# reesque/SfmFromScratch

Measured on AMD Instinct MI355X. Metric: images/sec detect+describe+match, 1080p, 1/2/4/8 MI355X, higher is better.
Workload: dtype f32; 1 GPU; BASELINE configs[1]: 32x 1080p per GPU, ScaleRotInvSIFT 4-level x2 octave pyramid, k=2500, fw 18, NNRatio 0.85 over consecutive pairs; frames_per_gpu=32, pairs_per_gpu=31, distinct_batches=2, parallelism=image-shard x1, batches_in_flight=2

## Files before the change

include/sfmfeat.h:

```cpp
#ifndef SFMFEAT_H_
#define SFMFEAT_H_

#include <stddef.h>
#include <stdint.h>

#ifdef __cplusplus
extern "C" {
#endif

#define SFM_OK 0
#define SFM_EINVAL 1
#define SFM_ESTATE 2
#define SFM_EDEVICE 3
#define SFM_ERANGE 4
#define SFM_EINDEX 5

#define SFM_MODE_SCALEROT 0
#define SFM_MODE_NAIVE 1

#define SFM_DESC_DIM 128
#define SFM_MAX_GAUSS 15
#define SFM_MAX_KSIZE 31
#define SFM_MAX_FW 64
#define SFM_MAX_LEVELS 12
// ... 198 lines not shown

int32_t sfm_debug_nms(int32_t device, const float* R, int32_t B, int32_t H, int32_t W, int32_t ksize,
                      const uint32_t* tnms, int32_t tile, uint64_t* keys_out, int64_t* counts_out);

float sfm_debug_time_harris(int32_t device, int32_t abl, int32_t B, int32_t H, int32_t W,
                            int32_t iters);
float sfm_debug_harris_stamps(int32_t device, int32_t abl, int32_t B, int32_t H, int32_t W,
                              int32_t iters, uint64_t* out, int64_t cap);

int64_t sfm_debug_match_stamps(uint64_t* out, int64_t cap);

int32_t sfm_debug_match_operands(sfm_ctx* ctx, int32_t slot, int64_t rows, uint16_t* hi, uint16_t* lo,
                                 float* norm2, float* rnorm, float* pmax);
int32_t sfm_debug_match_windows(sfm_ctx* ctx, int32_t pair, int64_t rows, int32_t* cand_n, float* cand_thr,
                                uint32_t* cand);

int32_t sfm_copy_wg(void* dst, const void* src, int64_t bytes, int32_t workgroups, void* stream);

int32_t sfm_debug_select_stats(sfm_ctx* ctx, int32_t* fallback_planes, int32_t* total_planes);
int32_t sfm_debug_pose_candidates(sfm_ctx* ctx, int32_t* cand_idx, int64_t entries);
int32_t sfm_debug_ransac_fits(sfm_ctx* ctx, double* F, int32_t* counts, int64_t entries);
int32_t sfm_debug_copy_level(sfm_ctx* ctx, int32_t l, int32_t what, float* out, void* stream);


#ifdef __cplusplus
}
#endif

#endif
```

sfmfromscratch_amd/_abi.py:

```python
from __future__ import annotations

import ctypes

import numpy as np

SFM_OK = 0
SFM_EINVAL = 1
SFM_ESTATE = 2
SFM_EDEVICE = 3
SFM_ERANGE = 4
SFM_EINDEX = 5

SFM_MODE_SCALEROT = 0
SFM_MODE_NAIVE = 1

SFM_DESC_DIM = 128
SFM_MAX_GAUSS = 15
SFM_MAX_KSIZE = 31
SFM_MAX_FW = 64
SFM_MAX_LEVELS = 12
SFM_BA_MAX_CAMERAS = 256
SFM_BA_MAX_POINTS = 1 << 24
SFM_BA_MAX_OBSERVATIONS = 1 << 26
SFM_TRACKS_MAX_NODES = 1 << 30

_vp = ctypes.c_void_p
TRACK_SIGNATURES = {
    "sfm_build_tracks_dev": (ctypes.c_int32, [_vp, _vp, ctypes.c_int32, ctypes.c_int64, _vp, ctypes.c_int32, _vp,
                                              _vp, _vp, ctypes.c_int32, _vp, _vp, _vp, _vp, _vp, _vp]),
    "sfm_triangulate_tracks_dev": (ctypes.c_int32, [_vp, _vp, _vp, _vp, ctypes.c_int32, ctypes.c_int32, _vp,
                                                    ctypes.c_int32, ctypes.c_int64, _vp, _vp, ctypes.c_int32, _vp,
                                                    _vp, _vp]),
}


MATCH_DEBUG_SIGNATURES = {
    "sfm_debug_match_operands": (ctypes.c_int32, [_vp, ctypes.c_int32, ctypes.c_int64, _vp, _vp, _vp, _vp, _vp]),
    "sfm_debug_match_windows": (ctypes.c_int32, [_vp, ctypes.c_int32, ctypes.c_int64, _vp, _vp, _vp]),
}
GEOM_DEBUG_SIGNATURES = {
    "sfm_debug_geom": (ctypes.c_int32, [ctypes.c_int32, ctypes.c_int32, _vp, ctypes.c_int64, _vp]),
}
(SFM_GEOM_RODRIGUES, SFM_GEOM_RODRIGUES_INV, SFM_GEOM_EIG3, SFM_GEOM_NULL4, SFM_GEOM_COMPOSE, SFM_GEOM_ROTATE,
 SFM_GEOM_WAVE_SUM, SFM_GEOM_BLOCK_SUM) = range(8)
GEOM_ROW_IN = (3, 9, 6, 16, 18, 12, 64, 512)
GEOM_ROW_OUT = (9, 3, 12, 4, 9, 3, 64, 512)
SFM_GEOM_MAX_ROWS = 1 << 20
MATCH_CAND_CAP = 256
MATCH_PREP_ROWS = 16


class SfmParams(ctypes.Structure):
    _fields_ = [
# ... 52 lines not shown
```

sfmfromscratch_amd/_native.py:

```python
from __future__ import annotations

import ctypes
import os
import sys
import threading

import numpy as np

from . import _abi
from ._abi import SfmParams

_HERE = os.path.dirname(os.path.abspath(__file__))
LIB_PATH = os.environ.get("SFMFEAT_LIB", os.path.join(_HERE, "lib", "libsfmfeat.so"))

_lib = None
_lib_lock = threading.Lock()

_fp = ctypes.POINTER(ctypes.c_float)
_i64p = ctypes.POINTER(ctypes.c_int64)
_i32p = ctypes.POINTER(ctypes.c_int32)
_u8p = ctypes.POINTER(ctypes.c_uint8)
_dp = ctypes.POINTER(ctypes.c_double)
_vp = ctypes.c_void_p

# ... 396 lines not shown
        pmax = np.empty((capP // _abi.MATCH_PREP_ROWS, 2), np.float32)
        check(self.lib.sfm_debug_match_operands(self.handle, int(slot), capP, hi.ctypes.data, lo.ctypes.data,
                                                norm2.ctypes.data, rnorm.ctypes.data, pmax.ctypes.data),
              self.handle)
        return hi, lo, norm2, rnorm, pmax

    def match_windows(self, pair: int, rows: int):
        rows = int(rows)
        cn = np.empty(max(rows, 1), np.int32)
        ct = np.empty(max(rows, 1), np.float32)
        cd = np.empty((max(rows, 1), _abi.MATCH_CAND_CAP), np.uint32)
        check(self.lib.sfm_debug_match_windows(self.handle, int(pair), rows, cn.ctypes.data, ct.ctypes.data,
                                               cd.ctypes.data), self.handle)
        return cn, ct, cd

    def _tensor_ptr(self, t, dtype: str, numel: int, what: str, optional: bool = False):
        if t is None:
            if optional:
                return None
            raise ValueError(f"{what} is required")
        if not (hasattr(t, "data_ptr") and hasattr(t, "is_cuda")):
            raise ValueError(f"{what} must be a device tensor")
        if not t.is_cuda or (t.device.index or 0) != self.device:
            raise ValueError(f"{what} must live on cuda:{self.device} (the context's device), not {t.device}")
        if str(t.dtype) != "torch." + dtype:
            raise ValueError(f"{what} must be {dtype}, not {t.dtype}")
        if not t.is_contiguous():
            raise ValueError(f"{what} must be contiguous")
        if t.numel() < numel:
            raise ValueError(f"{what} has {t.numel()} elements, fewer than {numel}")
# ... 200 lines not shown
```

sfmfromscratch_amd/csrc/api_match.hip:

```cpp
#include "ctx.h"

using namespace sfm;

namespace {

constexpr int kFusedPrepSpare = 8;

int64_t operand_rows(const sfm_ctx* c, int64_t cap) {
  return c->match.direct ? (cap + 63) / 64 * 64 : (cap + 127) / 128 * 128;
}

int operands_claim(sfm_ctx* c, const float* desc, const int32_t* count, int64_t cap, int nimg) {
  MatchOperandsWs& o = c->match.ops;
  const int64_t capP = operand_rows(c, cap);
  const size_t rows = (size_t)nimg * capP;
  struct {
    DevBuf& b;
    size_t bytes;
  } mfma[] = {{o.hi, rows * 128 * 2}, {o.lo, rows * 128 * 2}, {o.norm2, rows * 4}, {o.rnorm, rows * 4},
              {o.imgmax, (size_t)nimg * match_pmax_bytes(capP)}},
    direct[] = {{o.descT, rows * 128 * 4}};
  bool fits = true;
  if (c->match.direct) {
    for (auto& e : direct) fits = fits && e.b.bytes >= e.bytes;
// ... 51 lines not shown
               const int32_t* pairs, int P, float ratio, int32_t* matches, float* conf,
               int32_t* nmatch, hipStream_t st, bool prep = true) {
  if (P <= 0) return SFM_OK;
  if (cap < 1 || cap > kMaxMatchRows)
    return set_err(c, SFM_EINVAL, "match capacity must be in [1, 16384]");
  int rc;
  MatchWs& m = c->match;
  MatchOperandsWs& o = m.ops;
  if (prep) {
    if ((rc = match_prep_range(c, desc, count, nimg, cap, 0, nimg, st, true))) return rc;
  } else {
    if (o.desc != desc || o.count != count || o.prep_nimg != nimg || o.cap != cap)
      return set_err(c, SFM_ESTATE, "sfm_match_pairs_prepped_dev: this table was not the last one prepped "
                                    "(sfm_match_prep_dev) on this context");
  }
  const size_t per_pair = (size_t)cap * (sizeof(RowBest) + sizeof(int2) + (m.direct ? 0 : kMatchCandCap * 4 + 8));
  const int Pmax = (int)std::max<size_t>(
      1, std::min<size_t>(std::min<size_t>((size_t)P, m.budget / per_pair), (size_t)1 << kMatchUnitPairBits));
  if ((rc = ensure(c, m.rows, (size_t)Pmax * cap * sizeof(RowBest)))) return rc;
  if ((rc = ensure(c, m.ovf, (size_t)Pmax * cap * sizeof(int2)))) return rc;
  if (m.ovfc.bytes == 0) {
    if ((rc = ensure(c, m.ovfc, 16))) return rc;
    HIPCHK(c, hipMemsetAsync(m.ovfc.p, 0, 16, st));
  }
  if (!m.direct) {
    if ((rc = ensure(c, m.cand, (size_t)Pmax * cap * kMatchCandCap * 4))) return rc;
    if ((rc = ensure(c, m.candn, (size_t)Pmax * cap * 4))) return rc;
    if ((rc = ensure(c, m.candt, (size_t)Pmax * cap * 4))) return rc;
    if ((rc = ensure(c, m.units, match_units_words(Pmax, (int)cap) * 4))) return rc;
  }
  const int64_t capP = operand_rows(c, cap);
  const bool skip_sweep = (extract_switches().skip & 8) != 0;
  m.last_P = P;
  m.last_cap = cap;
  m.last_subs = (P + Pmax - 1) / Pmax;
  for (int p0 = 0; p0 < P; p0 += Pmax, ++m.calls) {
    const int Pn = std::min(Pmax, P - p0);
    const int32_t* pr = pairs + 2 * (int64_t)p0;
    {
      StageScope sc(c, SFM_PROF_MATCH, st);
      if (m.direct)
        launch_match_rows(as<float>(o.descT), count, capP, pr, Pn, ratio, as<RowBest>(m.rows), (int)cap, st);
      else if (!(m.calls > 0 && skip_sweep))
        launch_match_mfma(desc, count, cap, capP, as<_Float16>(o.hi), as<_Float16>(o.lo), as<float>(o.norm2),
                          as<float>(o.rnorm), o.imgmax.p, pr, Pn, ratio, as<RowBest>(m.rows), (int)cap,
                          as<uint32_t>(m.cand), as<int32_t>(m.candn), as<float>(m.candt), as<int>(m.ovfc),
                          as<int2>(m.ovf), as<int32_t>(m.units), st);
    }
    {
      StageScope sc(c, SFM_PROF_MATCH_POST, st);
      launch_match_compact(as<RowBest>(m.rows), count, pr, Pn, (int)cap, cap, matches + (int64_t)p0 * cap * 2,
                           conf + (int64_t)p0 * cap, nmatch + p0, m.direct ? nullptr : as<int>(m.ovfc), st);
    }
  }
  HIPCHK(c, hipGetLastError());
  return SFM_OK;
}

}

int operands_fused_begin(sfm_ctx* c, const float* desc, const int32_t* count, int64_t cap, int B,
                         MatchOperands* mo) {
// ... 115 lines not shown
  MatchWs& m = c->match;
  if (m.direct) return set_err(c, SFM_ESTATE, "the direct matcher keeps no windows");
  if (m.last_subs != 1)
    return set_err(c, SFM_ESTATE, m.last_subs ? "the last match call ran as more than one sub-launch"
                                              : "no match call on this context yet");
  if (pair >= m.last_P || rows > m.last_cap) return set_err(c, SFM_EINVAL, "pair or rows outside the last match call");
  HIPCHK(c, hipSetDevice(c->device));
  HIPCHK(c, hipDeviceSynchronize());
  const size_t r0 = (size_t)pair * (size_t)m.last_cap, n = (size_t)rows;
  HIPCHK(c, hipMemcpy(cand_n, as<int32_t>(m.candn) + r0, n * 4, hipMemcpyDeviceToHost));
  HIPCHK(c, hipMemcpy(cand_thr, as<float>(m.candt) + r0, n * 4, hipMemcpyDeviceToHost));
  HIPCHK(c, hipMemcpy(cand, as<uint32_t>(m.cand) + r0 * kMatchCandCap, n * kMatchCandCap * 4, hipMemcpyDeviceToHost));
  return SFM_OK;
}

}
```

sfmfromscratch_amd/csrc/ctx.h:

```cpp
#pragma once

#include <stdlib.h>
#include <string.h>

#include <algorithm>
#include <string>
#include <utility>
#include <vector>

#include "../../include/sfmfeat.h"
#include "extract_layout.h"
#include "kernels.h"

struct DevBuf {
  void* p = nullptr;
  size_t bytes = 0;
  DevBuf() = default;
  DevBuf(const DevBuf&) = delete;
  DevBuf& operator=(const DevBuf&) = delete;
  DevBuf(DevBuf&& o) noexcept : p(o.p), bytes(o.bytes) { o.p = nullptr, o.bytes = 0; }
  DevBuf& operator=(DevBuf&& o) noexcept {
    if (this != &o) {
      release();
      std::swap(p, o.p);
// ... 59 lines not shown
  int last_B = 0, last_H = 0, last_W = 0;
};

struct MatchOperandsWs {
  DevBuf hi, lo, norm2, rnorm, imgmax;
  DevBuf descT;
  const float* desc = nullptr;
  const int32_t* count = nullptr;
  int64_t cap = -1;
  int fused_B = 0;
  int prep_nimg = -1;
};

struct MatchWs {
  MatchOperandsWs ops;
  DevBuf rows, ovf, ovfc, cand, candn, candt, units;
  DevBuf h_desc, h_count, h_pairs, h_matches, h_conf, h_nmatch;
  bool fused_prep = false;
  bool direct = false;
  size_t budget = (size_t)4096 << 20;
  int64_t calls = 0;
  int last_P = 0, last_subs = 0;
  int64_t last_cap = 0;
};

struct IngestWs {
  DevBuf tab_h, tab_v, tmp, rgb, gray;
  DevBuf colmap, sets;
  int w = -1, w2 = -1, h = -1, h2 = -1, ksh = 0, ksv = 0, nsets = 0;
  bool rows = false;
  std::vector<int32_t> th, tv;
// ... 146 lines not shown
```

sfmfromscratch_amd/csrc/kernels.h:

```cpp
#pragma once

#include <hip/hip_runtime.h>
#include <stdint.h>

#include <vector>

#include "common.h"

namespace sfm {

#define SFM_NMS_MAX_HALF 15

constexpr int kHistBits = 12;
constexpr int kHistBins = 1 << kHistBits;
constexpr int kMedBits1 = 11;
constexpr int kMedBins1 = 1 << kMedBits1;
constexpr int kTopkLdsCap = 8192;
constexpr int kMaxMatchRows = 16384;
constexpr int kMatchCandCap = 256;
constexpr int kCounterStride = 32;
constexpr int kMatchUnitPairBits = 20;

constexpr float kMatchScale = 256.0f;
constexpr float kMatchLoScale = 2048.0f;
// ... 322 lines not shown
void launch_transpose_desc(const float* desc, const int32_t* count, int nimg, int64_t cap,
                           int64_t capP, float* descT, hipStream_t st);
void launch_match_rows(const float* descT, const int32_t* count, int64_t capP, const int32_t* pairs,
                       int P, float ratio, RowBest* rows, int max_rows, hipStream_t st);
void launch_match_compact(const RowBest* rows, const int32_t* count, const int32_t* pairs, int P,
                          int max_rows, int64_t cap, int32_t* matches, float* conf, int32_t* nmatch,
                          int* reset_counter, hipStream_t st);
void init_match_attributes(int max_rows);
size_t match_pmax_bytes(int64_t capP);
void launch_match_prep(const float* desc, const int32_t* count, int nimg, int64_t cap, int64_t capP,
                       _Float16* hi, _Float16* lo, float* norm2, float* rnorm, void* pmax, hipStream_t st);
void launch_match_mfma(const float* desc, const int32_t* count, int64_t cap, int64_t capP,
                       const _Float16* hi, const _Float16* lo, const float* norm2, const float* rnorm,
                       const void* pmax, const int32_t* pairs, int P, float ratio,
                       RowBest* rows, int max_rows, uint32_t* cand, int32_t* cand_n, float* cand_thr,
                       int* ovf_count, int2* ovf_list, int32_t* units, hipStream_t st);

}
```

sfmfromscratch_amd/csrc/match_mfma.hip:

```cpp
#include <stdlib.h>

#include <type_traits>

#include "kernels.h"

namespace sfm {

typedef _Float16 h8 __attribute__((ext_vector_type(8)));
typedef float f32x16 __attribute__((ext_vector_type(16)));

constexpr int kQW = 32;
constexpr int kWaves = 8;
constexpr int kQB = kQW * kWaves;
constexpr int kNT = 64 * kWaves;
constexpr int kRowH = 128 + 8;
constexpr int kCandCap = kMatchCandCap;
constexpr int kHalfCap = kCandCap / 2;
constexpr float kScale = kMatchScale;
constexpr float kLoScale = kMatchLoScale;

__global__ void __launch_bounds__(256) k_match_prep(const float* __restrict__ desc,
                                                   const int32_t* __restrict__ count, int64_t cap,
                                                   int64_t capP, _Float16* __restrict__ hi,
                                                   _Float16* __restrict__ lo,
// ... 89 lines not shown

SFM_DEV float other_half(float x) {
  const auto r = __builtin_amdgcn_permlane32_swap(__float_as_uint(x), __float_as_uint(x), false, false);
  return __uint_as_float((threadIdx.x & 32) ? r[0] : r[1]);
}
SFM_DEV int other_half(int x) { return __float_as_int(other_half(__int_as_float(x))); }

SFM_DEV void top2_merge(float& b1, int& j1, float& b2, float ob1, int oj1, float ob2) {
  if (ob1 < b1 || (ob1 == b1 && oj1 < j1)) {
    b2 = fminf(b1, ob2);
    b1 = ob1;
    j1 = oj1;
  } else {
    b2 = fminf(b2, ob1);
  }
}

constexpr int kTT2 = 64;
constexpr int kDmaBufs = 3, kDmaNormBufs = 4;
constexpr int kRegBufs = 2, kRegNormBufs = 3;
constexpr size_t kDBytes = (size_t)kWaves * 64 * 16 * 4;
constexpr size_t kSweepLds = (size_t)kDmaBufs * 2 * kTT2 * 256 + kDmaNormBufs * kTT2 * 4 + kDBytes;
static_assert(kSweepLds >= (size_t)kRegBufs * 2 * kTT2 * kRowH * 2 + kRegNormBufs * kTT2 * 4 + kDBytes,
              "one LDS array serves both staging forms");
static_assert(kSweepLds <= 160 * 1024, "LDS per CU");
constexpr int kWaves3 = 4;
constexpr size_t kSweepLds3 = (size_t)2 * 2 * kTT2 * 256 + 3 * kTT2 * 4 + 256;
static_assert(kSweepLds3 <= 80 * 1024, "half-CU sweep: at most half of the CU's LDS");
constexpr int sweep_waves(int stage) { return stage == 3 ? kWaves3 : kWaves; }
constexpr int sweep_rows(int stage) { return kQW * sweep_waves(stage); }
// ... 3 lines not shown
  asm volatile("s_mov_b32 %0, m0\n\ts_mov_b32 m0, %2\n\ts_nop 0\n\tglobal_load_lds_dwordx4 %1, off\n\ts_mov_b32 m0, %0"
               : "=&s"(keep)
               : "v"(gsrc), "s"(lds_dst)
               : "memory");
}
__device__ __forceinline__ void glds_x1(const void* gsrc, uint32_t lds_dst) {
  uint32_t keep;
  asm volatile("s_mov_b32 %0, m0\n\ts_mov_b32 m0, %2\n\ts_nop 0\n\tglobal_load_lds_dword %1, off\n\ts_mov_b32 m0, %0"
               : "=&s"(keep)
               : "v"(gsrc), "s"(lds_dst)
               : "memory");
}

__global__ void __launch_bounds__(1024) k_match_units(const int32_t* __restrict__ count,
                                                      const int32_t* __restrict__ pairs, int P, int max_rows,
                                                      int qbr, int32_t* __restrict__ units) {
  __shared__ uint32_t s_w[16];
  const int tid = threadIdx.x, lane = tid & 63, wid = tid >> 6;
  uint32_t base = 0;
  for (int c0 = 0; c0 < P; c0 += 1024) {
    const int p = c0 + tid;
    uint32_t q = 0;
    if (p < P) {
      const int n1 = min(count[pairs[2 * p]], max_rows), n2 = count[pairs[2 * p + 1]];
      q = (n1 > 0 && n2 > 0) ? (uint32_t)((n1 + qbr - 1) / qbr) : 0u;
    }
    const uint32_t x = wave_inclusive_scan(q);
    if (lane == 63) s_w[wid] = x;
    __syncthreads();
    uint32_t before = 0, tot = 0;
    for (int w = 0; w < 16; ++w) {
      const uint32_t t = s_w[w];
      before += w < wid ? t : 0u;
      tot += t;
    }
    const uint32_t first = base + before + x - q;
    for (uint32_t j = 0; j < q; ++j) units[1 + first + j] = (int32_t)((uint32_t)p | (j << kMatchUnitPairBits));
    base += tot;
    __syncthreads();
  }
  if (tid == 0) units[0] = (int32_t)base;
}

constexpr int kStampWg = 16, kStampSt = 40;
__device__ uint64_t g_match_stamps[kStampWg][kWaves][kStampSt + 1][4];
constexpr int kStampAll = 1024;
__device__ uint64_t g_match_wg[kStampAll][4];

template <int STAGE, int ABL = 0>
__global__ void __launch_bounds__(64 * sweep_waves(STAGE), STAGE == 3 ? 2 : 1) k_match_mfma(
    const int32_t* __restrict__ count, int64_t capP, const _Float16* __restrict__ hi,
    const _Float16* __restrict__ lo, const float* __restrict__ norm2, const float* __restrict__ rnorm,
    const float2* __restrict__ pmax, const int32_t* __restrict__ pairs, int P, int max_rows,
    uint32_t* __restrict__ cand, int32_t* __restrict__ cand_n, float* __restrict__ cand_thr,
    int* __restrict__ ovf_count, int2* __restrict__ ovf_list, const int32_t* __restrict__ units) {
  constexpr bool DMA = STAGE >= 1;
  constexpr bool H3 = STAGE == 3;
  constexpr int NW = sweep_waves(STAGE), NTH = 64 * NW, QBR = sweep_rows(STAGE);
  constexpr int NBUF = H3 ? 2 : DMA ? kDmaBufs : kRegBufs;
  constexpr int NNB = H3 ? 3 : DMA ? kDmaNormBufs : kRegNormBufs;
  constexpr int ROWB = DMA ? 256 : kRowH * 2;
  constexpr int ARRB = kTT2 * ROWB;
  constexpr int BUFB = 2 * ARRB;
  constexpr int OFF_N = NBUF * BUFB;
  constexpr int OFF_D = OFF_N + NNB * kTT2 * 4;
  constexpr size_t LDSB = H3 ? kSweepLds3 : kSweepLds;
  static_assert((size_t)OFF_D + (H3 ? 256 : kDBytes) <= LDSB, "LDS carve");
  __shared__ __attribute__((aligned(16))) unsigned char smem[LDSB];
  float* const sNb = reinterpret_cast<float*>(smem + OFF_N);
  float* const sDb = reinterpret_cast<float*>(smem + OFF_D);
// ... 25 lines not shown
    p = code & ((1 << kMatchUnitPairBits) - 1);
    row0 = (code >> kMatchUnitPairBits) * QBR;
  } else {
    p = grp + 8 * (slot8 / QB);
    row0 = (slot8 % QB) * QBR;
    if (p >= P) return;
  }
  const int tid = threadIdx.x, lane = tid & 63, wid = tid >> 6;
  const int i1 = pairs[2 * p], i2 = pairs[2 * p + 1];
  const int n1 = count[i1], n2 = count[i2];
  if (row0 >= n1 || n2 < 1) return;

  const int ql = wid * kQW + (lane & 31);
  const int qi = row0 + ql;
  const int half = lane >> 5;
  const int64_t qo = ((int64_t)i1 * capP + qi) * 128;
  h8 qhi[8], qlo[8];
#pragma unroll
  for (int kk = 0; kk < 8; ++kk) {
    qhi[kk] = *reinterpret_cast<const h8*>(hi + qo + kk * 16 + 8 * half);
    qlo[kk] = *reinterpret_cast<const h8*>(lo + qo + kk * 16 + 8 * half);
  }
  const float na = norm2[(int64_t)i1 * capP + qi];
  const float ra = rnorm[(int64_t)i1 * capP + qi];
  float maxn2, maxrn;
  {
    const int nblk = (int)(capP / kPrepRows);
    float m2 = 0.0f, mr = 0.0f;
    for (int t = tid; t < nblk; t += NTH) {
      const float2 v = pmax[(int64_t)i2 * nblk + t];
      m2 = fmaxf(m2, v.x);
      mr = fmaxf(mr, v.y);
    }
    for (int off = 32; off >= 1; off >>= 1) {
      m2 = fmaxf(m2, __shfl_xor(m2, off));
      mr = fmaxf(mr, __shfl_xor(mr, off));
    }
    if (lane == 0) {
      sDb[2 * wid] = m2;
// ... 333 lines not shown
  if constexpr (DMA) asm volatile("s_waitcnt vmcnt(0)" ::: "memory");
  if constexpr (STAMP) {
    if (tid == 0 && blockIdx.x < kStampAll) {
      g_match_wg[blockIdx.x][1] = __builtin_amdgcn_s_memrealtime();
      g_match_wg[blockIdx.x][3] = (uint64_t)p | ((uint64_t)row0 << 32);
    }
    if (lane == 0) s_stamp[(wid * (kStampSt + 1) + kStampSt) * 4 + 2] = __builtin_amdgcn_s_memrealtime();
    if (blockIdx.x < kStampWg) {
      __builtin_amdgcn_s_waitcnt(0xc07f);
      const uint64_t* src = s_stamp + wid * (kStampSt + 1) * 4;
      uint64_t* dst = &g_match_stamps[blockIdx.x][wid][0][0];
      for (int i = lane; i < (kStampSt + 1) * 4; i += 64) dst[i] = src[i];
    }
  }
  const float ob1 = other_half(b1), ob2 = other_half(b2);
  const float thr_final = fminf(fminf(fmaxf(b1, ob1), fminf(b2, ob2)) + E2, thr_w);
  const int ocnt = other_half(cnt);
  const bool unbounded = !(E2 <= 3.0e38f);
  if (live && half == 0) {
    cand_thr[(int64_t)p * max_rows + qi] = thr_final;
    cand_n[(int64_t)p * max_rows + qi] = unbounded ? 0x7fff : cnt | (ocnt << 16);
    if (cnt > kHalfCap || ocnt > kHalfCap || unbounded) {
      const int k = atomicAdd(ovf_count, 1);
      ovf_list[k] = make_int2(p, qi);
    }
  }
}

__global__ void __launch_bounds__(256) k_match_rerank(const float* __restrict__ desc,
                                                      const int32_t* __restrict__ count, int64_t cap,
                                                      const int32_t* __restrict__ pairs, int P, float ratio,
                                                      int max_rows, const uint32_t* __restrict__ cand,
                                                      const int32_t* __restrict__ cand_n,
                                                      const float* __restrict__ cand_thr,
                                                      RowBest* __restrict__ rows_out) {
  __shared__ uint16_t sJ[4][kCandCap];
  const int lane = threadIdx.x & 63, wv = threadIdx.x >> 6;
  const int grp = lane >> 3, l8 = lane & 7;
  const int64_t w = (int64_t)blockIdx.x * 4 + wv;
  const int p = (int)(w / max_rows), row = (int)(w % max_rows);
  if (p >= P) return;
  const int i1 = pairs[2 * p], i2 = pairs[2 * p + 1];
  const int n1 = count[i1], n2 = count[i2];
  if (row >= n1 || n2 < 1) return;
  const int cw = cand_n[w];
  const int c0 = cw & 0xffff, c1 = cw >> 16;
  if (c0 > kHalfCap || c1 > kHalfCap) return;
  const float thr = cand_thr[w];
  const uint32_t* list = cand + w * kCandCap;
  const float* A = desc + ((int64_t)i1 * cap + row) * 128;
  const float* Bd = desc + (int64_t)i2 * cap * 128;
  float a[16];
#pragma unroll
  for (int i = 0; i < 16; ++i) a[i] = A[8 * i + l8];
  int nk = 0;
  static_assert(kHalfCap % 64 == 0, "whole wavefront passes per half-list");
#pragma unroll
  for (int h = 0; h < 2; ++h) {
    const int ch = h ? c1 : c0;
// ... 43 lines not shown
    const float d1 = sqrtf(e1), d2 = sqrtf(e2);
    if (d2 > 0.0f) {
      const float nndr = d1 / d2;
      if (nndr <= ratio) { rb.col = j1; rb.nndr = nndr; }
    }
    rows_out[w] = rb;
  }
}

__global__ void __launch_bounds__(256) k_match_rerank2(const float* __restrict__ desc,
                                                       const int32_t* __restrict__ count, int64_t cap,
                                                       const int32_t* __restrict__ pairs, int P, float ratio,
                                                       int max_rows, const uint32_t* __restrict__ cand,
                                                       const int32_t* __restrict__ cand_n,
                                                       const float* __restrict__ cand_thr,
                                                       RowBest* __restrict__ rows_out) {
  __shared__ uint16_t sJ[4][2][kCandCap];
  const int lane = threadIdx.x & 63, wv = threadIdx.x >> 6, hf = lane >> 5, hl = lane & 31;
  const int grp = hl >> 3, l8 = lane & 7;
  const int64_t w = ((int64_t)blockIdx.x * 4 + wv) * 2 + hf;
  const int p = (int)(w / max_rows), row = (int)(w % max_rows);
  bool ok = p < P;
  int i1 = 0, i2 = 0, n1 = 0, n2 = 0;
  if (ok) {
    i1 = pairs[2 * p];
    i2 = pairs[2 * p + 1];
    n1 = count[i1];
    n2 = count[i2];
    ok = row < n1 && n2 >= 1;
  }
  int c0 = 0, c1 = 0;
  float thr = 0.0f;
  if (ok) {
    const int cw = cand_n[w];
    c0 = cw & 0xffff;
    c1 = cw >> 16;
    ok = c0 <= kHalfCap && c1 <= kHalfCap;
    thr = cand_thr[w];
  }
  const uint32_t* list = cand + w * kCandCap;
  const float* A = desc + ((int64_t)i1 * cap + row) * 128;
  const float* Bd = desc + (int64_t)i2 * cap * 128;
  float a[16];
#pragma unroll
  for (int i = 0; i < 16; ++i) a[i] = ok ? A[8 * i + l8] : 0.0f;
// ... 53 lines not shown
      const float nndr = d1 / d2;
      if (nndr <= ratio) { rb.col = j1; rb.nndr = nndr; }
    }
    rows_out[w] = rb;
  }
}

constexpr int kRrRows = 8;
constexpr int kRerank8MaxPairs = 0;
__global__ void __launch_bounds__(256) k_match_rerank8(const float* __restrict__ desc,
                                                      const int32_t* __restrict__ count, int64_t cap,
                                                      const int32_t* __restrict__ pairs, int P, float ratio,
                                                      int max_rows, const uint32_t* __restrict__ cand,
                                                      const int32_t* __restrict__ cand_n,
                                                      const float* __restrict__ cand_thr,
                                                      RowBest* __restrict__ rows_out) {
  __shared__ __attribute__((aligned(16))) float sA[4][kRrRows][128];
  __shared__ uint16_t sL[4][kRrRows * kCandCap];
  __shared__ float sDist[4][kRrRows * kCandCap];
  __shared__ int sBeg[4][kRrRows + 1];
  const int lane = threadIdx.x & 63, wv = threadIdx.x >> 6;
  const int grp = lane >> 3, l8 = lane & 7;
  const int64_t total = (int64_t)P * max_rows;
  const int64_t w0 = ((int64_t)blockIdx.x * 4 + wv) * kRrRows;
  if (w0 >= total) return;
  int c_l = 0, ok_l = 0, i1_l = 0, i2_l = 0, row_l = 0, p_l = 0;
  float thr_l = 0.0f;
  if (lane < kRrRows) {
    const int64_t w = w0 + lane;
    if (w < total) {
      p_l = (int)(w / max_rows);
      row_l = (int)(w % max_rows);
      i1_l = pairs[2 * p_l];
      i2_l = pairs[2 * p_l + 1];
      const int n1 = count[i1_l], n2 = count[i2_l];
      if (row_l < n1 && n2 >= 1) {
        c_l = cand_n[w];
        thr_l = cand_thr[w];
        ok_l = ((c_l & 0xffff) <= kHalfCap && (c_l >> 16) <= kHalfCap) ? 1 : 0;
      }
    }
    if (!ok_l) c_l = 0;
  }
#pragma unroll
  for (int q = 0; q < 4; ++q) {
    const int e = lane * 4 + 256 * q;
    const int r = e >> 7, k = e & 127;
    const int ir = __shfl(i1_l, r), rr = __shfl(row_l, r), okr = __shfl(ok_l, r);
    float4 v = make_float4(0.0f, 0.0f, 0.0f, 0.0f);
    if (okr) v = *reinterpret_cast<const float4*>(desc + ((int64_t)ir * cap + rr) * 128 + k);
    *reinterpret_cast<float4*>(&sA[wv][r][k]) = v;
  }
  const uint32_t* lists = cand + w0 * kCandCap;
  int nk = 0;
#pragma unroll 4
  for (int sidx = 0; sidx < kRrRows * kCandCap / 64; ++sidx) {
    const int e = sidx * 64 + lane;
    const int r = e / kCandCap, pos = e % kCandCap;
    const int cr = __shfl(c_l, r);
    const float tr = __shfl(thr_l, r);
    const int crh = pos < kHalfCap ? (cr & 0xffff) : (cr >> 16);
    const bool valid = (pos & (kHalfCap - 1)) < crh && w0 + r < total;
    const uint32_t ent = valid ? lists[e] : 0u;
    const bool keep = valid && __uint_as_float(ent & 0xffff0000u) <= tr;
    const uint64_t bal = __ballot(keep);
    if (pos == 0 && lane == (sidx * 64) % 64 && (e % kCandCap) == 0) sBeg[wv][r] = nk;
    if (keep) sL[wv][nk + __popcll(bal & ((1ull << lane) - 1ull))] = (uint16_t)(ent & 0xffffu);
    nk += __popcll(bal);
  }
  if (lane == 0) sBeg[wv][kRrRows] = nk;
  __builtin_amdgcn_wave_barrier();
  for (int s0 = 0; s0 < nk; s0 += 8) {
    const int s = s0 + grp;
    const bool ok = s < nk;
    const int j = ok ? (int)sL[wv][s] : 0;
    int r = 0;
#pragma unroll
    for (int k = 1; k < kRrRows; ++k) r += (s >= sBeg[wv][k]) ? 1 : 0;
// ... 19 lines not shown
    const int beg = sBeg[wv][lane], end = lane + 1 < kRrRows ? sBeg[wv][lane + 1] : nk;
    for (int s = beg; s < end; ++s) {
      const float dd = sDist[wv][s];
      const int j = (int)sL[wv][s];
      if (dd < e1 || (dd == e1 && j < j1)) { e2 = e1; e1 = dd; j1 = j; }
      else if (dd < e2) e2 = dd;
    }
    RowBest rb;
    rb.col = -1;
    rb.nndr = 0.0f;
    const float d1 = sqrtf(e1), d2 = sqrtf(e2);
    if (d2 > 0.0f) {
      const float nndr = d1 / d2;
      if (nndr <= ratio) { rb.col = j1; rb.nndr = nndr; }
    }
    rows_out[w0 + lane] = rb;
  }
}

__global__ void __launch_bounds__(256) k_match_overflow(const float* __restrict__ desc,
                                                        const int32_t* __restrict__ count, int64_t cap,
                                                        const int32_t* __restrict__ pairs, float ratio,
                                                        RowBest* __restrict__ rows_out, int max_rows,
                                                        const int* __restrict__ ovf_count,
                                                        const int2* __restrict__ ovf_list) {
  const int nov = *ovf_count;
  const int lane = threadIdx.x & 63;
  for (int w = blockIdx.x * 4 + (threadIdx.x >> 6); w < nov; w += gridDim.x * 4) {
    const int2 ent = ovf_list[w];
    const int p = ent.x, row = ent.y;
    const int i1 = pairs[2 * p], i2 = pairs[2 * p + 1];
// ... 31 lines not shown
  return 1 + (size_t)P * ((max_rows + sweep_rows(3) - 1) / sweep_rows(3));
}

size_t match_pmax_bytes(int64_t capP) { return (size_t)(capP / kPrepRows) * sizeof(float2); }

void launch_match_prep(const float* desc, const int32_t* count, int nimg, int64_t cap, int64_t capP,
                       _Float16* hi, _Float16* lo, float* norm2, float* rnorm, void* pmax, hipStream_t st) {
  hipLaunchKernelGGL(k_match_prep, dim3((unsigned)(capP / kPrepRows), nimg), dim3(256), 0, st, desc, count, cap,
                     capP, hi, lo, norm2, rnorm, static_cast<float2*>(pmax));
}

void launch_match_mfma(const float* desc, const int32_t* count, int64_t cap, int64_t capP,
                       const _Float16* hi, const _Float16* lo, const float* norm2, const float* rnorm,
                       const void* pmax, const int32_t* pairs, int P, float ratio,
                       RowBest* rows, int max_rows, uint32_t* cand, int32_t* cand_n, float* cand_thr,
                       int* ovf_count, int2* ovf_list, int32_t* units, hipStream_t st) {
  static const int stage = [] {
    const char* e = getenv("SFMFEAT_MATCH_STAGE");
    return (e && e[0] == 'r') ? 0 : (e && e[0] == '1') ? 1 : 3;
  }();
  static const int rr8_max = [] {
    const char* e = SFM_DIAG_ENV("SFMFEAT_RERANK8_MAX");
    return e ? atoi(e) : kRerank8MaxPairs;
  }();
  static const bool use_units = [] {
    const char* e = SFM_DIAG_ENV("SFMFEAT_MATCH_UNITS");
    return !(e && e[0] == '0');
  }();
  const int qbr = stage == 3 ? sweep_rows(3) : kQB;
  const int qb = (max_rows + qbr - 1) / qbr;
  const dim3 grid((unsigned)(8 * ((P + 7) / 8) * qb));
  if (!use_units) units = nullptr;
  if (units) hipLaunchKernelGGL(k_match_units, dim3(1), dim3(1024), 0, st, count, pairs, P, max_rows, qbr, units);
#define SFM_SWEEP(A, ABL)                                                                             \
  hipLaunchKernelGGL((k_match_mfma<A, ABL>), grid, dim3(64 * sweep_waves(A)), 0, st, count, capP, hi, lo,  \
                     norm2, rnorm,                                                                         \
                     static_cast<const float2*>(pmax), pairs, P, max_rows, cand, cand_n, cand_thr, ovf_count, \
                     ovf_list, units)
  static const int abl = [] {
    const char* e = SFM_ABLATION_ENV("SFMFEAT_MATCH_ABL");
    return e ? atoi(e) : 0;
  }();
#ifdef SFM_ABLATIONS
  switch (abl) {
    case 1: SFM_SWEEP(1, 1); break;
    case 2: SFM_SWEEP(1, 2); break;
    case 3: SFM_SWEEP(1, 3); break;
    case 4: SFM_SWEEP(1, 4); break;
    case 6: SFM_SWEEP(1, 6); break;
    case 16: SFM_SWEEP(1, 16); break;
    case 17: SFM_SWEEP(1, 17); break;
    case 32: SFM_SWEEP(1, 32); break;
    default: if (stage == 0) SFM_SWEEP(0, 0); else if (stage == 3) SFM_SWEEP(3, 0); else SFM_SWEEP(1, 0);
// ... 2 lines not shown
  (void)abl;
  if (stage == 0)
    SFM_SWEEP(0, 0);
  else if (stage == 3)
    SFM_SWEEP(3, 0);
  else
    SFM_SWEEP(1, 0);
#endif
#undef SFM_SWEEP
  static const int rr2 = [] {
    const char* e = getenv("SFMFEAT_RERANK2");
    return e ? atoi(e) : 1;
  }();
  if (rr2 && P > rr8_max)
    hipLaunchKernelGGL(k_match_rerank2, dim3((unsigned)(((int64_t)P * max_rows + 7) / 8)), dim3(256), 0, st, desc,
                       count, cap, pairs, P, ratio, max_rows, cand, cand_n, cand_thr, rows);
  else if (P <= rr8_max)
    hipLaunchKernelGGL(k_match_rerank8, dim3((unsigned)(((int64_t)P * max_rows + 4 * kRrRows - 1) / (4 * kRrRows))),
                       dim3(256), 0, st, desc, count, cap, pairs, P, ratio, max_rows, cand, cand_n, cand_thr, rows);
  else
    hipLaunchKernelGGL(k_match_rerank, dim3((unsigned)(((int64_t)P * max_rows + 3) / 4)), dim3(256), 0, st, desc,
                       count, cap, pairs, P, ratio, max_rows, cand, cand_n, cand_thr, rows);
  hipLaunchKernelGGL(k_match_overflow, dim3(256), dim3(256), 0, st, desc, count, cap, pairs, ratio, rows, max_rows,
                     ovf_count, ovf_list);
}

int64_t match_stamps_copy(uint64_t* out, int64_t cap) {
#ifdef SFM_ABLATIONS
  const int64_t n1 = (int64_t)sizeof(g_match_stamps) / 8, n = n1 + (int64_t)sizeof(g_match_wg) / 8;
  if (cap < n) return -1;
  if (hipMemcpyFromSymbol(out, HIP_SYMBOL(g_match_stamps), sizeof(g_match_stamps)) != hipSuccess) return -1;
  if (hipMemcpyFromSymbol(out + n1, HIP_SYMBOL(g_match_wg), sizeof(g_match_wg)) != hipSuccess) return -1;
  return n;
#else
  (void)out;
  (void)cap;
  return -1;
// ... 5 lines not shown
```

Before: 43570 images/sec.

## Skip provably unmatched rows in sweep and compact rerank work list

The MFMA sweep now checks, using the sweep's approximate best and second-best distances and their error bound, whether a row cannot pass the ratio test; such rows get a no-match result written directly. Remaining rows are appended to a compacted work list through wave-level ballot and atomics, and the rerank kernels walk that list instead of every (pair,row) slot. This cuts exact rerank work and idle waves, at the cost of extra atomics, a per-row skip byte buffer, and indirect candidate loads. Rerank grids stay sized for the full row count, so the extra blocks exit early.

```diff
diff --git a/include/sfmfeat.h b/include/sfmfeat.h
--- a/include/sfmfeat.h
+++ b/include/sfmfeat.h
@@ -236,6 +236,7 @@
                                  float* norm2, float* rnorm, float* pmax);
 int32_t sfm_debug_match_windows(sfm_ctx* ctx, int32_t pair, int64_t rows, int32_t* cand_n, float* cand_thr,
                                 uint32_t* cand);
+int32_t sfm_debug_match_skips(sfm_ctx* ctx, int32_t pair, int64_t rows, uint8_t* skip);
 
 int32_t sfm_copy_wg(void* dst, const void* src, int64_t bytes, int32_t workgroups, void* stream);
 
diff --git a/sfmfromscratch_amd/_abi.py b/sfmfromscratch_amd/_abi.py
--- a/sfmfromscratch_amd/_abi.py
+++ b/sfmfromscratch_amd/_abi.py
@@ -37,6 +37,7 @@
 MATCH_DEBUG_SIGNATURES = {
     "sfm_debug_match_operands": (ctypes.c_int32, [_vp, ctypes.c_int32, ctypes.c_int64, _vp, _vp, _vp, _vp, _vp]),
     "sfm_debug_match_windows": (ctypes.c_int32, [_vp, ctypes.c_int32, ctypes.c_int64, _vp, _vp, _vp]),
+    "sfm_debug_match_skips": (ctypes.c_int32, [_vp, ctypes.c_int32, ctypes.c_int64, _vp]),
 }
 GEOM_DEBUG_SIGNATURES = {
     "sfm_debug_geom": (ctypes.c_int32, [ctypes.c_int32, ctypes.c_int32, _vp, ctypes.c_int64, _vp]),
diff --git a/sfmfromscratch_amd/_native.py b/sfmfromscratch_amd/_native.py
--- a/sfmfromscratch_amd/_native.py
+++ b/sfmfromscratch_amd/_native.py
@@ -434,6 +434,12 @@
                                                cd.ctypes.data), self.handle)
         return cn, ct, cd
 
+    def match_skips(self, pair: int, rows: int):
+        rows = int(rows)
+        sk = np.empty(max(rows, 1), np.uint8)
+        check(self.lib.sfm_debug_match_skips(self.handle, int(pair), rows, sk.ctypes.data), self.handle)
+        return sk
+
     def _tensor_ptr(self, t, dtype: str, numel: int, what: str, optional: bool = False):
         if t is None:
             if optional:
diff --git a/sfmfromscratch_amd/csrc/api_match.hip b/sfmfromscratch_amd/csrc/api_match.hip
--- a/sfmfromscratch_amd/csrc/api_match.hip
+++ b/sfmfromscratch_amd/csrc/api_match.hip
@@ -89,9 +89,11 @@
       return set_err(c, SFM_ESTATE, "sfm_match_pairs_prepped_dev: this table was not the last one prepped "
                                     "(sfm_match_prep_dev) on this context");
   }
-  const size_t per_pair = (size_t)cap * (sizeof(RowBest) + sizeof(int2) + (m.direct ? 0 : kMatchCandCap * 4 + 8));
+  const size_t per_pair = (size_t)cap * (sizeof(RowBest) + sizeof(int2) + (m.direct ? 0 : kMatchCandCap * 4 + 13));
   const int Pmax = (int)std::max<size_t>(
-      1, std::min<size_t>(std::min<size_t>((size_t)P, m.budget / per_pair), (size_t)1 << kMatchUnitPairBits));
+      1, std::min<size_t>(std::min<size_t>(std::min<size_t>((size_t)P, m.budget / per_pair),
+                                           (size_t)1 << kMatchUnitPairBits),
+                          (size_t)0x7fffffff / (size_t)cap));
   if ((rc = ensure(c, m.rows, (size_t)Pmax * cap * sizeof(RowBest)))) return rc;
   if ((rc = ensure(c, m.ovf, (size_t)Pmax * cap * sizeof(int2)))) return rc;
   if (m.ovfc.bytes == 0) {
@@ -102,6 +104,8 @@
     if ((rc = ensure(c, m.cand, (size_t)Pmax * cap * kMatchCandCap * 4))) return rc;
     if ((rc = ensure(c, m.candn, (size_t)Pmax * cap * 4))) return rc;
     if ((rc = ensure(c, m.candt, (size_t)Pmax * cap * 4))) return rc;
+    if ((rc = ensure(c, m.cands, (size_t)Pmax * cap))) return rc;
+    if ((rc = ensure(c, m.work, (size_t)Pmax * cap * 4))) return rc;
     if ((rc = ensure(c, m.units, match_units_words(Pmax, (int)cap) * 4))) return rc;
   }
   const int64_t capP = operand_rows(c, cap);
@@ -119,8 +123,8 @@
       else if (!(m.calls > 0 && skip_sweep))
         launch_match_mfma(desc, count, cap, capP, as<_Float16>(o.hi), as<_Float16>(o.lo), as<float>(o.norm2),
                           as<float>(o.rnorm), o.imgmax.p, pr, Pn, ratio, as<RowBest>(m.rows), (int)cap,
-                          as<uint32_t>(m.cand), as<int32_t>(m.candn), as<float>(m.candt), as<int>(m.ovfc),
-                          as<int2>(m.ovf), as<int32_t>(m.units), st);
+                          as<uint32_t>(m.cand), as<int32_t>(m.candn), as<float>(m.candt), as<uint8_t>(m.cands),
+                          as<uint32_t>(m.work), as<int>(m.ovfc), as<int2>(m.ovf), as<int32_t>(m.units), st);
     }
     {
       StageScope sc(c, SFM_PROF_MATCH_POST, st);
@@ -266,4 +270,19 @@
   return SFM_OK;
 }
 
-}
+int32_t sfm_debug_match_skips(sfm_ctx* c, int32_t pair, int64_t rows, uint8_t* skip) {
+  if (!c || !skip || pair < 0 || rows < 1) return SFM_EINVAL;
+  MatchWs& m = c->match;
+  if (m.direct) return set_err(c, SFM_ESTATE, "the direct matcher keeps no windows");
+  if (m.last_subs != 1)
+    return set_err(c, SFM_ESTATE, m.last_subs ? "the last match call ran as more than one sub-launch"
+                                              : "no match call on this context yet");
+  if (pair >= m.last_P || rows > m.last_cap) return set_err(c, SFM_EINVAL, "pair or rows outside the last match call");
+  HIPCHK(c, hipSetDevice(c->device));
+  HIPCHK(c, hipDeviceSynchronize());
+  HIPCHK(c, hipMemcpy(skip, as<uint8_t>(m.cands) + (size_t)pair * (size_t)m.last_cap, (size_t)rows,
+                      hipMemcpyDeviceToHost));
+  return SFM_OK;
+}
+
+}
diff --git a/sfmfromscratch_amd/csrc/ctx.h b/sfmfromscratch_amd/csrc/ctx.h
--- a/sfmfromscratch_amd/csrc/ctx.h
+++ b/sfmfromscratch_amd/csrc/ctx.h
@@ -97,7 +97,7 @@
 
 struct MatchWs {
   MatchOperandsWs ops;
-  DevBuf rows, ovf, ovfc, cand, candn, candt, units;
+  DevBuf rows, ovf, ovfc, cand, candn, candt, cands, work, units;
   DevBuf h_desc, h_count, h_pairs, h_matches, h_conf, h_nmatch;
   bool fused_prep = false;
   bool direct = false;
diff --git a/sfmfromscratch_amd/csrc/kernels.h b/sfmfromscratch_amd/csrc/kernels.h
--- a/sfmfromscratch_amd/csrc/kernels.h
+++ b/sfmfromscratch_amd/csrc/kernels.h
@@ -360,6 +360,7 @@
                        const _Float16* hi, const _Float16* lo, const float* norm2, const float* rnorm,
                        const void* pmax, const int32_t* pairs, int P, float ratio,
                        RowBest* rows, int max_rows, uint32_t* cand, int32_t* cand_n, float* cand_thr,
-                       int* ovf_count, int2* ovf_list, int32_t* units, hipStream_t st);
+                       uint8_t* cand_skip, uint32_t* work_list, int* ovf_count, int2* ovf_list, int32_t* units,
+                       hipStream_t st);
 
 }
diff --git a/sfmfromscratch_amd/csrc/match_mfma.hip b/sfmfromscratch_amd/csrc/match_mfma.hip
--- a/sfmfromscratch_amd/csrc/match_mfma.hip
+++ b/sfmfromscratch_amd/csrc/match_mfma.hip
@@ -127,6 +127,16 @@
   } else {
     b2 = fminf(b2, ob1);
   }
+}
+
+SFM_DEV bool proven_unmatched(float r1, float r2, float E2, float ratio) {
+  const float E = 0.5f * E2;
+  float L = fmaxf(r1 - E, 0.0f);
+  if (L > 0.0f) L = __uint_as_float(__float_as_uint(L) - 1u);
+  float U = r2 + E;
+  if (U >= 0.0f) U = __uint_as_float((__float_as_uint(U) & 0x7fffffffu) + 1u);
+  const float t = sqrtf(L) / sqrtf(U);
+  return U > 0.0f && U < INFINITY && t > ratio;
 }
 
 constexpr int kTT2 = 64;
@@ -160,7 +170,8 @@
 
 __global__ void __launch_bounds__(1024) k_match_units(const int32_t* __restrict__ count,
                                                       const int32_t* __restrict__ pairs, int P, int max_rows,
-                                                      int qbr, int32_t* __restrict__ units) {
+                                                      int qbr, int32_t* __restrict__ units,
+                                                      int* __restrict__ work_count) {
   __shared__ uint32_t s_w[16];
   const int tid = threadIdx.x, lane = tid & 63, wid = tid >> 6;
   uint32_t base = 0;
@@ -185,7 +196,10 @@
     base += tot;
     __syncthreads();
   }
-  if (tid == 0) units[0] = (int32_t)base;
+  if (tid == 0) {
+    units[0] = (int32_t)base;
+    *work_count = 0;
+  }
 }
 
 constexpr int kStampWg = 16, kStampSt = 40;
@@ -199,7 +213,9 @@
     const _Float16* __restrict__ lo, const float* __restrict__ norm2, const float* __restrict__ rnorm,
     const float2* __restrict__ pmax, const int32_t* __restrict__ pairs, int P, int max_rows,
     uint32_t* __restrict__ cand, int32_t* __restrict__ cand_n, float* __restrict__ cand_thr,
-    int* __restrict__ ovf_count, int2* __restrict__ ovf_list, const int32_t* __restrict__ units) {
+    int* __restrict__ ovf_count, int2* __restrict__ ovf_list, const int32_t* __restrict__ units, float ratio,
+    uint8_t* __restrict__ cand_skip, RowBest* __restrict__ rows_out, int* __restrict__ work_count,
+    uint32_t* __restrict__ work_list) {
   constexpr bool DMA = STAGE >= 1;
   constexpr bool H3 = STAGE == 3;
   constexpr int NW = sweep_waves(STAGE), NTH = 64 * NW, QBR = sweep_rows(STAGE);
@@ -255,15 +271,16 @@
   const int ql = wid * kQW + (lane & 31);
   const int qi = row0 + ql;
   const int half = lane >> 5;
-  const int64_t qo = ((int64_t)i1 * capP + qi) * 128;
+  const int qr = min(qi, (int)capP - 1);
+  const int64_t qo = ((int64_t)i1 * capP + qr) * 128;
   h8 qhi[8], qlo[8];
 #pragma unroll
   for (int kk = 0; kk < 8; ++kk) {
     qhi[kk] = *reinterpret_cast<const h8*>(hi + qo + kk * 16 + 8 * half);
     qlo[kk] = *reinterpret_cast<const h8*>(lo + qo + kk * 16 + 8 * half);
   }
-  const float na = norm2[(int64_t)i1 * capP + qi];
-  const float ra = rnorm[(int64_t)i1 * capP + qi];
+  const float na = norm2[(int64_t)i1 * capP + qr];
+  const float ra = rnorm[(int64_t)i1 * capP + qr];
   float maxn2, maxrn;
   {
     const int nblk = (int)(capP / kPrepRows);
@@ -627,16 +644,36 @@
     }
   }
   const float ob1 = other_half(b1), ob2 = other_half(b2);
-  const float thr_final = fminf(fminf(fmaxf(b1, ob1), fminf(b2, ob2)) + E2, thr_w);
+  const float r2 = fminf(fmaxf(b1, ob1), fminf(b2, ob2));
+  const float thr_final = fminf(r2 + E2, thr_w);
   const int ocnt = other_half(cnt);
   const bool unbounded = !(E2 <= 3.0e38f);
+  bool todo = false;
   if (live && half == 0) {
     cand_thr[(int64_t)p * max_rows + qi] = thr_final;
     cand_n[(int64_t)p * max_rows + qi] = unbounded ? 0x7fff : cnt | (ocnt << 16);
-    if (cnt > kHalfCap || ocnt > kHalfCap || unbounded) {
+    const bool over = cnt > kHalfCap || ocnt > kHalfCap || unbounded;
+    if (over) {
       const int k = atomicAdd(ovf_count, 1);
       ovf_list[k] = make_int2(p, qi);
     }
+    const bool skip = !over && proven_unmatched(fminf(b1, ob1), r2, E2, ratio);
+    cand_skip[(int64_t)p * max_rows + qi] = skip ? 1 : 0;
+    if (skip) {
+      RowBest rb;
+      rb.col = -1;
+      rb.nndr = 0.0f;
+      rows_out[(int64_t)p * max_rows + qi] = rb;
+    }
+    todo = !over && !skip;
+  }
+  const uint64_t bal = __ballot(todo);
+  if (bal) {
+    const int lead = __ffsll((unsigned long long)bal) - 1;
+    int base = 0;
+    if (lane == lead) base = atomicAdd(work_count, __popcll(bal));
+    base = __shfl(base, lead);
+    if (todo) work_list[base + __popcll(bal & ((1ull << lane) - 1ull))] = (uint32_t)(p * max_rows + qi);
   }
 }
 
@@ -646,16 +683,17 @@
                                                       int max_rows, const uint32_t* __restrict__ cand,
                                                       const int32_t* __restrict__ cand_n,
                                                       const float* __restrict__ cand_thr,
+                                                      const int* __restrict__ work_count,
+                                                      const uint32_t* __restrict__ work_list,
                                                       RowBest* __restrict__ rows_out) {
   __shared__ uint16_t sJ[4][kCandCap];
   const int lane = threadIdx.x & 63, wv = threadIdx.x >> 6;
   const int grp = lane >> 3, l8 = lane & 7;
-  const int64_t w = (int64_t)blockIdx.x * 4 + wv;
+  const int64_t t = (int64_t)blockIdx.x * 4 + wv;
+  if (t >= *work_count) return;
+  const int64_t w = work_list[t];
   const int p = (int)(w / max_rows), row = (int)(w % max_rows);
-  if (p >= P) return;
   const int i1 = pairs[2 * p], i2 = pairs[2 * p + 1];
-  const int n1 = count[i1], n2 = count[i2];
-  if (row >= n1 || n2 < 1) return;
   const int cw = cand_n[w];
   const int c0 = cw & 0xffff, c1 = cw >> 16;
   if (c0 > kHalfCap || c1 > kHalfCap) return;
@@ -729,21 +767,18 @@
                                                        int max_rows, const uint32_t* __restrict__ cand,
                                                        const int32_t* __restrict__ cand_n,
                                                        const float* __restrict__ cand_thr,
+                                                       const int* __restrict__ work_count,
+                                                       const uint32_t* __restrict__ work_list,
                                                        RowBest* __restrict__ rows_out) {
   __shared__ uint16_t sJ[4][2][kCandCap];
   const int lane = threadIdx.x & 63, wv = threadIdx.x >> 6, hf = lane >> 5, hl = lane & 31;
   const int grp = hl >> 3, l8 = lane & 7;
-  const int64_t w = ((int64_t)blockIdx.x * 4 + wv) * 2 + hf;
+  const int64_t t = ((int64_t)blockIdx.x * 4 + wv) * 2 + hf;
+  bool ok = t < *work_count;
+  if (!__any(ok)) return;
+  const int64_t w = ok ? (int64_t)work_list[t] : 0;
   const int p = (int)(w / max_rows), row = (int)(w % max_rows);
-  bool ok = p < P;
-  int i1 = 0, i2 = 0, n1 = 0, n2 = 0;
-  if (ok) {
-    i1 = pairs[2 * p];
-    i2 = pairs[2 * p + 1];
-    n1 = count[i1];
-    n2 = count[i2];
-    ok = row < n1 && n2 >= 1;
-  }
+  const int i1 = pairs[2 * p], i2 = pairs[2 * p + 1];
   int c0 = 0, c1 = 0;
   float thr = 0.0f;
   if (ok) {
@@ -827,6 +862,8 @@
                                                       int max_rows, const uint32_t* __restrict__ cand,
                                                       const int32_t* __restrict__ cand_n,
                                                       const float* __restrict__ cand_thr,
+                                                      const int* __restrict__ work_count,
+                                                      const uint32_t* __restrict__ work_list,
                                                       RowBest* __restrict__ rows_out) {
   __shared__ __attribute__((aligned(16))) float sA[4][kRrRows][128];
   __shared__ uint16_t sL[4][kRrRows * kCandCap];
@@ -834,24 +871,21 @@
   __shared__ int sBeg[4][kRrRows + 1];
   const int lane = threadIdx.x & 63, wv = threadIdx.x >> 6;
   const int grp = lane >> 3, l8 = lane & 7;
-  const int64_t total = (int64_t)P * max_rows;
-  const int64_t w0 = ((int64_t)blockIdx.x * 4 + wv) * kRrRows;
-  if (w0 >= total) return;
-  int c_l = 0, ok_l = 0, i1_l = 0, i2_l = 0, row_l = 0, p_l = 0;
+  const int64_t total = *work_count;
+  const int64_t t0 = ((int64_t)blockIdx.x * 4 + wv) * kRrRows;
+  if (t0 >= total) return;
+  int c_l = 0, ok_l = 0, w_l = 0, i1_l = 0, i2_l = 0, row_l = 0, p_l = 0;
   float thr_l = 0.0f;
   if (lane < kRrRows) {
-    const int64_t w = w0 + lane;
-    if (w < total) {
-      p_l = (int)(w / max_rows);
-      row_l = (int)(w % max_rows);
+    if (t0 + lane < total) {
+      w_l = (int)work_list[t0 + lane];
+      p_l = w_l / max_rows;
+      row_l = w_l % max_rows;
       i1_l = pairs[2 * p_l];
       i2_l = pairs[2 * p_l + 1];
-      const int n1 = count[i1_l], n2 = count[i2_l];
-      if (row_l < n1 && n2 >= 1) {
-        c_l = cand_n[w];
-        thr_l = cand_thr[w];
-        ok_l = ((c_l & 0xffff) <= kHalfCap && (c_l >> 16) <= kHalfCap) ? 1 : 0;
-      }
+      c_l = cand_n[w_l];
+      thr_l = cand_thr[w_l];
+      ok_l = ((c_l & 0xffff) <= kHalfCap && (c_l >> 16) <= kHalfCap) ? 1 : 0;
     }
     if (!ok_l) c_l = 0;
   }
@@ -864,7 +898,6 @@
     if (okr) v = *reinterpret_cast<const float4*>(desc + ((int64_t)ir * cap + rr) * 128 + k);
     *reinterpret_cast<float4*>(&sA[wv][r][k]) = v;
   }
-  const uint32_t* lists = cand + w0 * kCandCap;
   int nk = 0;
 #pragma unroll 4
   for (int sidx = 0; sidx < kRrRows * kCandCap / 64; ++sidx) {
@@ -873,8 +906,9 @@
     const int cr = __shfl(c_l, r);
     const float tr = __shfl(thr_l, r);
     const int crh = pos < kHalfCap ? (cr & 0xffff) : (cr >> 16);
-    const bool valid = (pos & (kHalfCap - 1)) < crh && w0 + r < total;
-    const uint32_t ent = valid ? lists[e] : 0u;
+    const int64_t wr = __shfl(w_l, r);
+    const bool valid = (pos & (kHalfCap - 1)) < crh;
+    const uint32_t ent = valid ? cand[wr * kCandCap + pos] : 0u;
     const bool keep = valid && __uint_as_float(ent & 0xffff0000u) <= tr;
     const uint64_t bal = __ballot(keep);
     if (pos == 0 && lane == (sidx * 64) % 64 && (e % kCandCap) == 0) sBeg[wv][r] = nk;
@@ -924,7 +958,7 @@
       const float nndr = d1 / d2;
       if (nndr <= ratio) { rb.col = j1; rb.nndr = nndr; }
     }
-    rows_out[w0 + lane] = rb;
+    rows_out[w_l] = rb;
   }
 }
 
@@ -986,7 +1020,8 @@
                        const _Float16* hi, const _Float16* lo, const float* norm2, const float* rnorm,
                        const void* pmax, const int32_t* pairs, int P, float ratio,
                        RowBest* rows, int max_rows, uint32_t* cand, int32_t* cand_n, float* cand_thr,
-                       int* ovf_count, int2* ovf_list, int32_t* units, hipStream_t st) {
+                       uint8_t* cand_skip, uint32_t* work_list, int* ovf_count, int2* ovf_list, int32_t* units,
+                       hipStream_t st) {
   static const int stage = [] {
     const char* e = getenv("SFMFEAT_MATCH_STAGE");
     return (e && e[0] == 'r') ? 0 : (e && e[0] == '1') ? 1 : 3;
@@ -999,16 +1034,20 @@
     const char* e = SFM_DIAG_ENV("SFMFEAT_MATCH_UNITS");
     return !(e && e[0] == '0');
   }();
+  int* const work_count = ovf_count + 1;
   const int qbr = stage == 3 ? sweep_rows(3) : kQB;
   const int qb = (max_rows + qbr - 1) / qbr;
   const dim3 grid((unsigned)(8 * ((P + 7) / 8) * qb));
   if (!use_units) units = nullptr;
-  if (units) hipLaunchKernelGGL(k_match_units, dim3(1), dim3(1024), 0, st, count, pairs, P, max_rows, qbr, units);
+  if (units)
+    hipLaunchKernelGGL(k_match_units, dim3(1), dim3(1024), 0, st, count, pairs, P, max_rows, qbr, units, work_count);
+  else
+    (void)hipMemsetAsync(work_count, 0, sizeof(int), st);
 #define SFM_SWEEP(A, ABL)                                                                             \
   hipLaunchKernelGGL((k_match_mfma<A, ABL>), grid, dim3(64 * sweep_waves(A)), 0, st, count, capP, hi, lo,  \
                      norm2, rnorm,                                                                         \
                      static_cast<const float2*>(pmax), pairs, P, max_rows, cand, cand_n, cand_thr, ovf_count, \
-                     ovf_list, units)
+                     ovf_list, units, ratio, cand_skip, rows, work_count, work_list)
   static const int abl = [] {
     const char* e = SFM_ABLATION_ENV("SFMFEAT_MATCH_ABL");
     return e ? atoi(e) : 0;
@@ -1041,13 +1080,16 @@
   }();
   if (rr2 && P > rr8_max)
     hipLaunchKernelGGL(k_match_rerank2, dim3((unsigned)(((int64_t)P * max_rows + 7) / 8)), dim3(256), 0, st, desc,
-                       count, cap, pairs, P, ratio, max_rows, cand, cand_n, cand_thr, rows);
+                       count, cap, pairs, P, ratio, max_rows, cand, cand_n, cand_thr, work_count,
+                       work_list, rows);
   else if (P <= rr8_max)
     hipLaunchKernelGGL(k_match_rerank8, dim3((unsigned)(((int64_t)P * max_rows + 4 * kRrRows - 1) / (4 * kRrRows))),
-                       dim3(256), 0, st, desc, count, cap, pairs, P, ratio, max_rows, cand, cand_n, cand_thr, rows);
+                       dim3(256), 0, st, desc, count, cap, pairs, P, ratio, max_rows, cand, cand_n, cand_thr, work_count,
+                       work_list, rows);
   else
     hipLaunchKernelGGL(k_match_rerank, dim3((unsigned)(((int64_t)P * max_rows + 3) / 4)), dim3(256), 0, st, desc,
-                       count, cap, pairs, P, ratio, max_rows, cand, cand_n, cand_thr, rows);
+                       count, cap, pairs, P, ratio, max_rows, cand, cand_n, cand_thr, work_count,
+                       work_list, rows);
   hipLaunchKernelGGL(k_match_overflow, dim3(256), dim3(256), 0, st, desc, count, cap, pairs, ratio, rows, max_rows,
                      ovf_count, ovf_list);
 }
```

New measurement: 44220 images/sec (median of 6 runs). 1.5% higher.
